# ilovepose/fast-human-pose-estimation.pytorch

Hardware: AMD Instinct MI355X
Metric: images/sec FPD train step (4-stack HG student, 8-stack teacher) 256x256 (higher is better)
Workload: dtype bf16; 1 GPU; configs[1]: hourglass student S=4 F=128 + teacher S=8 F=256, 256x256, batch 32/GPU, fused FPD step incl. Adam, teacher forward one batch ahead on a 2nd stream; global_batch=32, parallelism=dp1, backend=mfma, launch=one native plan call per phase, kernels launched eagerly on 3 streams, ranks=1, finite=True

## Files before the change

### fast-human-pose-estimation.pytorch_amd/csrc/bneck_fused.hip

```cpp
#include <algorithm>
#include <type_traits>

#include "conv_dispatch.h"
#include "fused_lds.h"
#include "fused_tile.h"

namespace {


#ifdef FPD_BNECK_TIMING
#define STAMP(i) do { if (tid == 0 && bid_in == 0) stamps[i] = clock64(); } while (0)
#else
#define STAMP(i) do { } while (0)
#endif

template <int P>
__device__ __forceinline__ void bneck_fold_tables(const fpd_bneck_t& a, float* out, int tid, int nthreads) {
    constexpr int C = 2 * P;
    for (int c = tid; c < C; c += nthreads) {
        float sc, sh;
        bn_coef_eval(a.bn1, c, sc, sh);
        out[c] = sc;
        out[C + c] = sh;
        out[2 * C + 4 * P + c] = a.b3 ? a.b3[c] : 0.f;
    }
    for (int c = tid; c < 2 * P; c += nthreads) {
        const bool second = c >= P;
        const int cc = second ? c - P : c;
        float sc, sh;
        bn_coef_eval(second ? a.bn3 : a.bn2, cc, sc, sh);
        const float* bias = second ? a.b2 : a.b1;
        out[2 * C + (second ? 2 * P : 0) + cc] = sc;
        out[2 * C + (second ? 2 * P : 0) + P + cc] = fmaf(sc, bias ? bias[cc] : 0.f, sh);
    }
}

template <int P>
__global__ void bneck_fold_kernel(const fpd_bneck_t a, float* out) { bneck_fold_tables<P>(a, out, threadIdx.x, blockDim.x); }

template <int P, bool UPADD>
__device__ __forceinline__ void bneck_eval_body(const fpd_bneck_t& a, const int logW, const int bid_in, const int nblk, const int ntiles) {
    using L = BneckLds<P>;
    constexpr int C = L::C, LDX = L::LDX, LD2 = L::LD2, CW = L::CW, ASTG = L::ASTG;
    constexpr int TNH = P / 64;
    constexpr int NSTEP = 9 + 2;
    constexpr int W1V = P * 8 / 512;
    constexpr int NCH = C / 64;
    extern __shared__ __attribute__((aligned(16))) unsigned char smem[];

    const int tid = threadIdx.x, lane = tid & 63, wave = tid >> 6;
#ifdef FPD_BNECK_TIMING
    long long stamps[8];
    long long astamp[10];
    int acnt = 0;
#define ASTAMP() do { if (tid == 0 && bid_in == 0 && acnt < 10) astamp[acnt++] = clock64(); } while (0)
#else
#define ASTAMP() do { } while (0)
#endif
    STAMP(0);
    const int q = wave & 3, hC = wave >> 2;
    const int koff = 8 * (lane >> 5);
    const int H = a.H, W = a.W;
    const int M = a.N * H * W, GR = a.N * H;
    const int nrows = 128 >> logW, hrows = nrows + 2, WP = W + 2;
    const int rrows = 2 * nrows;
    const bool whole = L::whole(H, W);
    const int irows = L::irows(whole, nrows);
    const int zero_px = irows * WP;
    int m0 = 0, g0 = 0;
    int vrow0 = 0;

    float* s_sc1 = reinterpret_cast<float*>(smem);
    float* s_sh1 = s_sc1 + C;
    float* s_sc2 = s_sh1 + C;
    float* s_sh2 = s_sc2 + P;
    float* s_sc3 = s_sh2 + P;
    float* s_sh3 = s_sc3 + P;
    float* s_b3 = s_sh3 + P;
    bf16_t* sA2 = reinterpret_cast<bf16_t*>(s_sc1 + L::TAB);
    bf16_t* sR2 = sA2 + L::image_px(irows, W) * LD2;
    const bf16_t* __restrict__ x = reinterpret_cast<const bf16_t*>(a.x);
    const bf16_t* __restrict__ x2 = reinterpret_cast<const bf16_t*>(UPADD ? a.x2 : nullptr);
    const bf16_t* __restrict__ w1 = reinterpret_cast<const bf16_t*>(a.w1);
    const bf16_t* __restrict__ w2 = reinterpret_cast<const bf16_t*>(a.w2);
    const bf16_t* __restrict__ w3 = reinterpret_cast<const bf16_t*>(a.w3);

    int hp0 = whole ? W : 0;
    int npass = whole ? 1 : ((hrows * W + 127) >> 7);
    const int xpx = tid >> 3, xcv = (tid & 7) * 8;
    int xo[2];
    int xo2[UPADD ? 2 : 1];
    bool xok[2];
    auto pass_addr = [&](int p) __attribute__((always_inline)) {
#pragma unroll
        for (int i = 0; i < 2; ++i) {
            const int hp = hp0 + 128 * p + xpx + 64 * i;
            const int hr = hp >> logW, j = hp & (W - 1);
            const int g = g0 - 1 + hr;
            xok[i] = hr < hrows && (unsigned)g < (unsigned)GR;
            xo[i] = xok[i] ? (g * W + j) * C + xcv : 0;
            if constexpr (UPADD) xo2[i] = xok[i] ? ((((g >> 1) << logW) >> 1) + (j >> 1)) * C + xcv : 0;
        }
    };
    int w1o[W1V], w1l[W1V];
#pragma unroll
    for (int i = 0; i < W1V; ++i) {
        const int v = tid + i * 512;
        w1o[i] = (v >> 3) * C + (v & 7) * 8;
        w1l[i] = 128 * LDX + (v >> 3) * LDX + (v & 7) * 8;
    }
    const int xl = xpx * LDX + xcv;

    u32x4 rx[NCH][2], rw[NCH][W1V];
    u32x4 rx2[UPADD ? NCH : 1][2];
    auto a_load = [&](auto kcc) __attribute__((always_inline)) {
        constexpr int kc = decltype(kcc)::value;
        static_for<2>([&](auto ic) {
            constexpr int i = decltype(ic)::value;
            const u32x4 z = {0u, 0u, 0u, 0u};
            rx[kc][i] = z;
            if (xok[i]) rx[kc][i] = *reinterpret_cast<const u32x4*>(x + (xo[i] + kc * 64));
            if constexpr (UPADD) {
                rx2[kc][i] = z;
                if (xok[i]) rx2[kc][i] = *reinterpret_cast<const u32x4*>(x2 + (xo2[i] + kc * 64));
            }
        });
        static_for<W1V>([&](auto ic) {
            constexpr int i = decltype(ic)::value;
            rw[kc][i] = *reinterpret_cast<const u32x4*>(w1 + (w1o[i] + kc * 64));
        });
    };
    auto a_sum = [&](auto kcc, auto ic) __attribute__((always_inline)) {
        constexpr int kc = decltype(kcc)::value, i = decltype(ic)::value;
        if constexpr (UPADD) rx[kc][i] = bf16x8_sum(rx[kc][i], rx2[kc][i]);
    };
    constexpr int NSL = 2 + W1V;
    auto a_store_slice = [&](auto kcc, auto slc) __attribute__((always_inline)) {
        constexpr int kc = decltype(kcc)::value, sl = decltype(slc)::value;
        bf16_t* dst = sR2 + (kc & 1) * ASTG;
        if constexpr (sl < 2) {
            f32x4 sc[2], sh[2];
            sc[0] = *reinterpret_cast<const f32x4*>(s_sc1 + kc * 64 + xcv);
            sc[1] = *reinterpret_cast<const f32x4*>(s_sc1 + kc * 64 + xcv + 4);
            sh[0] = *reinterpret_cast<const f32x4*>(s_sh1 + kc * 64 + xcv);
            sh[1] = *reinterpret_cast<const f32x4*>(s_sh1 + kc * 64 + xcv + 4);
            float f[8];
            const u32x4 r = rx[kc][sl];
            DT<bf16_t>::unpack(make_uint4(r[0], r[1], r[2], r[3]), f);
#pragma unroll
            for (int e = 0; e < 8; ++e) f[e] = fmaxf(fmaf(f[e], sc[e >> 2][e & 3], sh[e >> 2][e & 3]), 0.f);
            *reinterpret_cast<uint4*>(dst + xl + 64 * sl * LDX) = DT<bf16_t>::pack(f);
        } else if constexpr (sl < NSL) {
            *reinterpret_cast<u32x4*>(dst + w1l[sl - 2]) = rw[kc][sl - 2];
        }
    };
    auto a_store = [&](auto kcc) __attribute__((always_inline)) {
        static_for<NSL>([&](auto slc) { a_store_slice(kcc, slc); });
    };
    constexpr int CPR = P / 8;
    constexpr int RPI = 64 / CPR;
    constexpr int DPW = P / RPI / 8;
    unsigned dma2[DPW], dma3[DPW];
#pragma unroll
    for (int j = 0; j < DPW; ++j) {
        const int row = wave * DPW * RPI + j * RPI + lane / CPR;
        const int sw = (P == 128) ? (row & 15) : ((row >> 1) & 7);
        const int c8 = ((lane % CPR) ^ sw) * 8;
        dma2[j] = (unsigned)(row * 9 * P + c8) * 2u;
        dma3[j] = (unsigned)(row * P + c8) * 2u;
    }
    auto t_dma = [&](auto sc_) __attribute__((always_inline)) {
        constexpr int s = decltype(sc_)::value;
        unsigned char* ring = reinterpret_cast<unsigned char*>(sR2) + (s & 1) * L::RING * 2 + wave * DPW * 1024;
        const char* gbase = s < 9 ? reinterpret_cast<const char*>(w2) + s * P * 2
                                  : reinterpret_cast<const char*>(w3) + (s - 9) * P * P * 2;
        static_for<DPW>([&](auto jc) {
            constexpr int j = decltype(jc)::value;
            unsigned off = s < 9 ? dma2[j] : dma3[j];
            asm volatile("" : "+v"(off));
            __builtin_amdgcn_global_load_lds((const __attribute__((address_space(1))) void*)(gbase + off),
                                             (__attribute__((address_space(3))) void*)(ring + j * 1024), 16, 0, 0);
        });
    };

    if (a.folded != nullptr) {
        for (int v = tid; v < L::TAB / 4; v += 512)
            reinterpret_cast<f32x4*>(s_sc1)[v] = reinterpret_cast<const f32x4*>(a.folded)[v];
    } else {
        bneck_fold_tables<P>(a, s_sc1, tid, 512);
    }

    const int t_beg = fpd_cut(bid_in, ntiles, nblk), t_end = fpd_cut(bid_in + 1, ntiles, nblk);
    for (int tile = t_beg; tile < t_end; ++tile) {
    {
        m0 = tile * 128;
        g0 = m0 >> logW;
        vrow0 = (tile * nrows) % rrows;
        if (!whole) {
            const bool incr = tile > t_beg && (g0 % H) != 0;
            hp0 = incr ? 2 * W : 0;
            npass = incr ? 1 : ((hrows * W + 127) >> 7);
        }
    }
    pass_addr(0);
    static_for<NCH>([&](auto kcc) { a_load(kcc); });
    if (npass > 1) pass_addr(1);
    __syncthreads();
    {
        constexpr int VR = LD2 / 8;
        const uint4 z = make_uint4(0, 0, 0, 0);
        for (int v = tid; v < (2 * irows + 3) * VR; v += 512) {
            const int pz = v / VR, cv = (v - pz * VR) * 8;
            const int px = pz < 2 * irows ? ((pz >> 1) * WP + ((pz & 1) ? WP - 1 : 0)) : zero_px + (pz - 2 * irows);
            *reinterpret_cast<uint4*>(sA2 + px * LD2 + cv) = z;
        }
    }
    a_sum(std::integral_constant<int, 0>{}, std::integral_constant<int, 0>{});
    a_sum(std::integral_constant<int, 0>{}, std::integral_constant<int, 1>{});
    STAMP(1);

    auto refill = [&](auto kcc, int pp) __attribute__((always_inline)) {
        if (pp + 1 < npass) a_load(kcc);
    };
#ifdef FPD_BNECK_TIMING
    acnt = 0;
#endif
    ASTAMP();
    a_store(std::integral_constant<int, 0>{});
    refill(std::integral_constant<int, 0>{}, 0);
    __syncthreads();
    ASTAMP();
    for (int p = 0; p < npass; ++p) {
        f32x16 acc[TNH];
#pragma unroll
        for (int tn = 0; tn < TNH; ++tn)
#pragma unroll
            for (int i = 0; i < 16; ++i) acc[tn][i] = 0.f;
        static_for<NCH>([&](auto kcc) {
            constexpr int kc = decltype(kcc)::value;
            auto stage_slice = [&](auto slc, auto lastc) __attribute__((always_inline)) {
                constexpr bool last = decltype(lastc)::value;
                if constexpr (kc + 1 < NCH) {
                    a_store_slice(std::integral_constant<int, (kc + 1) % NCH>{}, slc);
                    if constexpr (last) refill(std::integral_constant<int, (kc + 1) % NCH>{}, p);
                } else {
                    if (p + 1 < npass) {
                        a_store_slice(std::integral_constant<int, 0>{}, slc);
                        if constexpr (last) {
                            if (p + 2 < npass) pass_addr(p + 2);
                            refill(std::integral_constant<int, 0>{}, p + 1);
                        }
                    }
                }
            };
            const bf16_t* xrow = sR2 + (kc & 1) * ASTG + (q * 32 + (lane & 31)) * LDX + koff;
            const bf16_t* wrow = sR2 + (kc & 1) * ASTG + 128 * LDX + (hC * CW + (lane & 31)) * LDX + koff;
            static_for<4>([&](auto kkc) {
                constexpr int kk = decltype(kkc)::value;
                const bf16x8 px = *reinterpret_cast<const bf16x8*>(xrow + kk * 16);
#pragma unroll
                for (int tn = 0; tn < TNH; ++tn) {
                    const bf16x8 wf = *reinterpret_cast<const bf16x8*>(wrow + tn * 32 * LDX + kk * 16);
                    acc[tn] = __builtin_amdgcn_mfma_f32_32x32x16_bf16(wf, px, acc[tn], 0, 0, 0);
                }
                if constexpr (!UPADD) {
                    stage_slice(kkc, std::integral_constant<bool, kk == NSL - 1>{});
                } else {
                    if constexpr (kk < 2) {
                        if constexpr (kc + 1 < NCH) {
                            if (p == 0) a_sum(std::integral_constant<int, (kc + 1) % NCH>{}, kkc);
                        }
                        stage_slice(std::integral_constant<int, (kk + 2 < NSL ? kk + 2 : NSL)>{}, std::false_type{});
                    } else {
                        stage_slice(std::integral_constant<int, kk - 2>{}, std::integral_constant<bool, kk == 3>{});
                        if (p + 1 < npass) a_sum(kcc, std::integral_constant<int, kk - 2>{});
                    }
                }
            });
            __syncthreads();
            ASTAMP();
        });
        if (p + 1 == npass) {
            t_dma(std::integral_constant<int, 0>{});
            t_dma(std::integral_constant<int, 1>{});
        }
        const int hp = hp0 + 128 * p + q * 32 + (lane & 31);
        const int hr = hp >> logW, j = hp & (W - 1);
        if (hr < hrows) {
            const int rr = whole ? hr : ((vrow0 + hr) & (rrows - 1));
            act_store(acc, s_sc2, s_sh2, hC * CW, lane, sA2 + (rr * WP + j + 1) * LD2);
        }
    }

    const int ml = q * 32 + (lane & 31);
    const int a3px = whole ? 0 : vrow0 * WP;
    int ab[3];
    {
        const int ti = ml >> logW, tj = ml & (W - 1);
        const int g = g0 + ti;
        const int pr = g % H;
        const bool live = g < GR;
        const int r0 = whole ? ti : ((vrow0 + ti) & (rrows - 1)), r1 = whole ? ti + 1 : ((vrow0 + ti + 1) & (rrows - 1)),
                  r2 = whole ? ti + 2 : ((vrow0 + ti + 2) & (rrows - 1));
        ab[0] = (live && pr - 1 >= 0) ? (r0 * WP + tj) * LD2 : zero_px * LD2;
        ab[1] = live ? (r1 * WP + tj) * LD2 : zero_px * LD2;
        ab[2] = (live && pr + 1 < H) ? (r2 * WP + tj) * LD2 : zero_px * LD2;
    }
    STAMP(2);
    __syncthreads();
    STAMP(3);

    f32x16 accB[TNH], accC[2][TNH];
#pragma unroll
    for (int tn = 0; tn < TNH; ++tn)
#pragma unroll
        for (int i = 0; i < 16; ++i) accB[tn][i] = 0.f;

    const int wsw = (P == 128) ? (lane & 15) : ((lane >> 1) & 7);
    auto mma = [&](const bf16_t* arow, int buf, f32x16* acc, auto behind) __attribute__((always_inline)) {
        const bf16_t* wbase = sR2 + buf * L::RING + (hC * CW + (lane & 31)) * P;
        static_for<P / 16>([&](auto kkc) {
            constexpr int kk = decltype(kkc)::value;
            const bf16x8 px = *reinterpret_cast<const bf16x8*>(arow + kk * 16);
            const int wo = ((2 * kk + (lane >> 5)) ^ wsw) * 8;
#pragma unroll
            for (int tn = 0; tn < TNH; ++tn) {
                const bf16x8 wf = *reinterpret_cast<const bf16x8*>(wbase + tn * 32 * P + wo);
                acc[tn] = __builtin_amdgcn_mfma_f32_32x32x16_bf16(wf, px, acc[tn], 0, 0, 0);
            }
            behind(kkc);
        });
    };

    constexpr int VW = CW / 8;
    constexpr int NIT = 32 * VW / 64;
    u32x4 rres[2][NIT];
    u32x4 rres2[UPADD ? NIT : 1];
    auto res_load = [&](auto stc) __attribute__((always_inline)) {
        constexpr int st = decltype(stc)::value;
        static_for<NIT>([&](auto itc) {
            constexpr int it = decltype(itc)::value;
            const int idx = lane + 64 * it;
            const int px = idx / VW, cv = (idx - px * VW) * 8;
            const int m = m0 + q * 32 + px;
            const u32x4 z = {0u, 0u, 0u, 0u};
            rres[st][it] = z;
            if (m < M) rres[st][it] = *reinterpret_cast<const u32x4*>(x + ((size_t)m * C + st * P + hC * CW + cv));
            if constexpr (UPADD) {
                const int g = m >> logW, j = m & (W - 1);
                const int m2 = (((g >> 1) << logW) >> 1) + (j >> 1);
                rres2[it] = z;
                if (m < M) rres2[it] = *reinterpret_cast<const u32x4*>(x2 + ((size_t)m2 * C + st * P + hC * CW + cv));
            }
        });
    };
    auto res_sum = [&](auto stc, auto itc) __attribute__((always_inline)) {
        constexpr int st = decltype(stc)::value, it = decltype(itc)::value;
        if constexpr (UPADD && it < NIT) rres[st][it] = bf16x8_sum(rres[st][it], rres2[it]);
    };

    static_for<NSTEP>([&](auto sc_) {
        constexpr int s = decltype(sc_)::value;
        if constexpr (s >= 1 && s + 1 < NSTEP) t_dma(std::integral_constant<int, (s + 1 < NSTEP ? s + 1 : 0)>{});
        if constexpr (s < 9) {
            mma(sA2 + ab[s / 3] + (s % 3) * LD2 + koff, s & 1, accB, [](auto) {});
        } else {
#pragma unroll
            for (int tn = 0; tn < TNH; ++tn)
#pragma unroll
                for (int i = 0; i < 16; ++i) accC[s - 9][tn][i] = 0.f;
            mma(sA2 + (a3px + ml) * LD2 + koff, s & 1, accC[s - 9],
                [&](auto kkc) { res_sum(std::integral_constant<int, s - 9>{}, kkc); });
        }
        if constexpr (s + 1 < NSTEP) {
            if constexpr (s == 8) res_load(std::integral_constant<int, 0>{});
            if constexpr (s == 9) res_load(std::integral_constant<int, 1>{});
            __syncthreads();
        }
        if constexpr (s == 8) {
            STAMP(4);
            act_store(accB, s_sc3, s_sh3, hC * CW, lane, sA2 + (a3px + ml) * LD2);
            __syncthreads();
        }
    });

    STAMP(5);
    float* stage = reinterpret_cast<float*>(sR2) + wave * 32 * L::LST;
    bf16_t* __restrict__ y = reinterpret_cast<bf16_t*>(a.y);
    static_for<2>([&](auto stc) {
        constexpr int st = decltype(stc)::value;
        __syncthreads();
        epi_stage<TNH>(accC[st], stage, lane);
        __syncthreads();
        static_for<NIT>([&](auto itc) {
            constexpr int it = decltype(itc)::value;
            const int idx = lane + 64 * it;
            const int px = idx / VW, cv = (idx - px * VW) * 8;
            const int m = m0 + q * 32 + px;
            if (m < M) {
                const int c = st * P + hC * CW + cv;
                *reinterpret_cast<uint4*>(y + ((size_t)m * C + c)) = epi_vec(stage + px * L::LST + cv, s_b3 + c, rres[st][it]);
            }
        });
    });
    }
#ifdef FPD_BNECK_TIMING
    STAMP(6);
    if (tid == 0 && bid_in == 0)
        printf("bneck W=%d: setup %lld | phaseA %lld | tile0 %lld | B(9 taps) %lld | a3+C %lld | epilogue %lld | total %lld cycles\n",
               W, stamps[1] - stamps[0], stamps[2] - stamps[1], stamps[3] - stamps[2], stamps[4] - stamps[3],
               stamps[5] - stamps[4], stamps[6] - stamps[5], stamps[6] - stamps[0]);
    if (tid == 0 && bid_in == 0 && acnt == 10)
        printf("  phase A steps: first-stage %lld | pass0 %lld %lld %lld %lld | pass1 %lld %lld %lld %lld | a2 write %lld\n",
               astamp[1] - astamp[0], astamp[2] - astamp[1], astamp[3] - astamp[2], astamp[4] - astamp[3], astamp[5] - astamp[4],
               astamp[6] - astamp[5], astamp[7] - astamp[6], astamp[8] - astamp[7], astamp[9] - astamp[8], stamps[2] - astamp[9]);
#endif
}

template <int P, bool UPADD>
__global__ __launch_bounds__(512, 1) void bneck_eval_kernel(const fpd_bneck_t a, const int logW, const int ntiles) {
    bneck_eval_body<P, UPADD>(a, logW, blockIdx.x, gridDim.x, ntiles);
}

template <int P>
__global__ __launch_bounds__(512, 1) void bneck_eval_pair_kernel(const fpd_bneck_t a, const fpd_bneck_t b, const int logWa,
                                                                 const int logWb, const int nblk_a, const int ntiles_a,
                                                                 const int ntiles_b) {
    if ((int)blockIdx.x < nblk_a) bneck_eval_body<P, false>(a, logWa, blockIdx.x, nblk_a, ntiles_a);
    else bneck_eval_body<P, false>(b, logWb, (int)blockIdx.x - nblk_a, (int)gridDim.x - nblk_a, ntiles_b);
}

static GridCap g_bneck_cap{"FPD_BNECK_BLOCKS", 128};

template <int P>
int launch_bneck_pair(const fpd_bneck_t& a, const fpd_bneck_t& b, hipStream_t st) {
    const size_t lds = std::max(BneckLds<P>::bytes(a.H, a.W), BneckLds<P>::bytes(b.H, b.W));
    static LdsAttr configured;
    if (int rc_ = configured.ensure(reinterpret_cast<const void*>(&bneck_eval_pair_kernel<P>), lds)) return rc_;
    int la = 0, lb = 0;
    while ((1 << la) < a.W) ++la;
    while ((1 << lb) < b.W) ++lb;
    const int ta = cdiv(a.N * a.H * a.W, 128), tb = cdiv(b.N * b.H * b.W, 128);
    int na = ta, nb = tb;
    const int cap = g_bneck_cap.get();
    if (ta + tb > cap) {
        const int capb = std::max(1, (int)((int64_t)cap * tb / (ta + tb)));
        nb = fpd_balanced_blocks(tb, capb);
        na = fpd_balanced_blocks(ta, std::max(1, cap - nb));
    }
    FPD_LAUNCH((bneck_eval_pair_kernel<P>), dim3(na + nb), dim3(512), lds, st, a, b, la, lb, na, ta, tb);
    return 0;
}

template <int P, bool UPADD>
int launch_bneck(const fpd_bneck_t& a, int logW, hipStream_t st) {
    const size_t lds = BneckLds<P>::bytes(a.H, a.W);
    static LdsAttr configured;
    if (int rc_ = configured.ensure(reinterpret_cast<const void*>(&bneck_eval_kernel<P, UPADD>), lds)) return rc_;
    const int ntiles = cdiv(a.N * a.H * a.W, 128);
    FPD_LAUNCH((bneck_eval_kernel<P, UPADD>), dim3(fpd_balanced_blocks(ntiles, g_bneck_cap.get())), dim3(512), lds, st, a, logW, ntiles);
    return 0;
}

}

int fpd_bneck_blocks_option(int value) { return g_bneck_cap.set(value); }

static bool bneck_in_domain(const fpd_bneck_t& a) {
    if (a.dtype != FPD_BF16 || a.C != 2 * a.P || (a.P != 64 && a.P != 128)) return false;
    if (a.W < 4 || a.W > 64 || (a.W & (a.W - 1)) != 0) return false;
    const int hw = a.H * a.W;
    return hw % 128 == 0 || 128 % hw == 0;
}

static EnvOpt g_bneck_upadd{"FPD_BNECK_UPADD", 1};
int fpd_bneck_upadd_option(int value) { return g_bneck_upadd.set(value < 0 ? 0 : value); }

const char* fpd_bneck_upadd_why_not(const fpd_bneck_t& a) {
    if (g_bneck_upadd.get() == 0) return "switched off (FPD_BNECK_UPADD=0 / option bneck_upadd)";
    if (!bneck_in_domain(a)) return "the shape is outside the fused kernel's domain";
    if (a.W < 8) return "W must be one of 8, 16, 32, 64";
    if (a.H & 1) return "H must be even";
    return nullptr;
}

int fpd_bneck_fused_launch(const fpd_bneck_t& a, hipStream_t st) {
    if (!bneck_in_domain(a)) return 1;
    int logW = 0;
    while ((1 << logW) < a.W) ++logW;
    if (a.x2 != nullptr) {
        if (fpd_bneck_upadd_why_not(a) != nullptr) return 1;
        return a.P == 128 ? launch_bneck<128, true>(a, logW, st) : launch_bneck<64, true>(a, logW, st);
    }
    return a.P == 128 ? launch_bneck<128, false>(a, logW, st) : launch_bneck<64, false>(a, logW, st);
}

int fpd_bneck_fused_pair_launch(const fpd_bneck_t& a, const fpd_bneck_t& b, hipStream_t st) {
    if (!bneck_in_domain(a) || !bneck_in_domain(b) || a.P != b.P || a.x2 != nullptr || b.x2 != nullptr) return 1;
    return a.P == 128 ? launch_bneck_pair<128>(a, b, st) : launch_bneck_pair<64>(a, b, st);
}

int fpd_bneck_fold_launch(const fpd_bneck_t& a, float* out, hipStream_t st) {
    if (a.C != 2 * a.P || (a.P != 64 && a.P != 128)) return 1;
    if (a.P == 128) FPD_LAUNCH((bneck_fold_kernel<128>), dim3(1), dim3(256), 0, st, a, out);
    else FPD_LAUNCH((bneck_fold_kernel<64>), dim3(1), dim3(256), 0, st, a, out);
    return 0;
}
```

Measured before the change: 3656 images/s.

## Software-pipeline LDS operand reads ahead of MFMA and use buffer loads for weight DMA

Double-buffers the bf16x8 operand fragments in both the 1x1 conv and the 3x3/1x1 tap loops, so reads for k-step kk+1 (and the next tap's first activation row) are issued before the MFMAs of step kk. sched_group_barrier hints interleave DS reads with MFMAs. The weight DMA switches from global_load_lds to buffer_load_lds with a resource descriptor and constant offsets, which reduces address VALU work. The trade-off is extra VGPR pressure, which is why the UPADD P=128 variant keeps the unpipelined path, and a prefetch across a __syncthreads boundary must read data that is already valid.

Result: no change. 3675 images/s, median of 6 (+0.5%).

```diff
diff --git a/fast-human-pose-estimation.pytorch_amd/csrc/bneck_fused.hip b/fast-human-pose-estimation.pytorch_amd/csrc/bneck_fused.hip
--- a/fast-human-pose-estimation.pytorch_amd/csrc/bneck_fused.hip
+++ b/fast-human-pose-estimation.pytorch_amd/csrc/bneck_fused.hip
@@ -46,6 +46,7 @@
     constexpr int NSTEP = 9 + 2;
     constexpr int W1V = P * 8 / 512;
     constexpr int NCH = C / 64;
+    constexpr bool APIPE = !(UPADD && P == 128);
     extern __shared__ __attribute__((aligned(16))) unsigned char smem[];
 
     const int tid = threadIdx.x, lane = tid & 63, wave = tid >> 6;
@@ -172,14 +173,13 @@
     auto t_dma = [&](auto sc_) __attribute__((always_inline)) {
         constexpr int s = decltype(sc_)::value;
         unsigned char* ring = reinterpret_cast<unsigned char*>(sR2) + (s & 1) * L::RING * 2 + wave * DPW * 1024;
-        const char* gbase = s < 9 ? reinterpret_cast<const char*>(w2) + s * P * 2
-                                  : reinterpret_cast<const char*>(w3) + (s - 9) * P * P * 2;
+        const auto rsrc = __builtin_amdgcn_make_buffer_rsrc(const_cast<bf16_t*>(s < 9 ? w2 : w3), 0, (s < 9 ? 9 * P * P : C * P) * 2, 0x00020000);
         static_for<DPW>([&](auto jc) {
             constexpr int j = decltype(jc)::value;
             unsigned off = s < 9 ? dma2[j] : dma3[j];
             asm volatile("" : "+v"(off));
-            __builtin_amdgcn_global_load_lds((const __attribute__((address_space(1))) void*)(gbase + off),
-                                             (__attribute__((address_space(3))) void*)(ring + j * 1024), 16, 0, 0);
+            __builtin_amdgcn_raw_ptr_buffer_load_lds(rsrc, (__attribute__((address_space(3))) void*)(ring + j * 1024), 16, (int)off,
+                                                     s < 9 ? s * P * 2 : (s - 9) * P * P * 2, 0, 0);
         });
     };
 
@@ -255,14 +255,21 @@
             };
             const bf16_t* xrow = sR2 + (kc & 1) * ASTG + (q * 32 + (lane & 31)) * LDX + koff;
             const bf16_t* wrow = sR2 + (kc & 1) * ASTG + 128 * LDX + (hC * CW + (lane & 31)) * LDX + koff;
+            bf16x8 apx[2], awf[2][TNH];
+            auto a_read = [&](auto kkc) __attribute__((always_inline)) {
+                constexpr int kk = decltype(kkc)::value;
+                apx[kk & 1] = *reinterpret_cast<const bf16x8*>(xrow + kk * 16);
+#pragma unroll
+                for (int tn = 0; tn < TNH; ++tn) awf[kk & 1][tn] = *reinterpret_cast<const bf16x8*>(wrow + tn * 32 * LDX + kk * 16);
+            };
+            if constexpr (APIPE) a_read(std::integral_constant<int, 0>{});
             static_for<4>([&](auto kkc) {
                 constexpr int kk = decltype(kkc)::value;
-                const bf16x8 px = *reinterpret_cast<const bf16x8*>(xrow + kk * 16);
-#pragma unroll
-                for (int tn = 0; tn < TNH; ++tn) {
-                    const bf16x8 wf = *reinterpret_cast<const bf16x8*>(wrow + tn * 32 * LDX + kk * 16);
-                    acc[tn] = __builtin_amdgcn_mfma_f32_32x32x16_bf16(wf, px, acc[tn], 0, 0, 0);
-                }
+                if constexpr (!APIPE) a_read(kkc);
+                else if constexpr (kk + 1 < 4) a_read(std::integral_constant<int, kk + 1>{});
+#pragma unroll
+                for (int tn = 0; tn < TNH; ++tn)
+                    acc[tn] = __builtin_amdgcn_mfma_f32_32x32x16_bf16(awf[kk & 1][tn], apx[kk & 1], acc[tn], 0, 0, 0);
                 if constexpr (!UPADD) {
                     stage_slice(kkc, std::integral_constant<bool, kk == NSL - 1>{});
                 } else {
@@ -317,17 +324,37 @@
         for (int i = 0; i < 16; ++i) accB[tn][i] = 0.f;
 
     const int wsw = (P == 128) ? (lane & 15) : ((lane >> 1) & 7);
-    auto mma = [&](const bf16_t* arow, int buf, f32x16* acc, auto behind) __attribute__((always_inline)) {
+    bf16x8 fpx[2], fwf[2][TNH];
+    auto px_read = [&](const bf16_t* arow, auto kkc) __attribute__((always_inline)) {
+        constexpr int kk = decltype(kkc)::value;
+        fpx[kk & 1] = *reinterpret_cast<const bf16x8*>(arow + kk * 16);
+    };
+    auto w_read = [&](const bf16_t* wbase, auto kkc) __attribute__((always_inline)) {
+        constexpr int kk = decltype(kkc)::value;
+        const int wo = ((2 * kk + (lane >> 5)) ^ wsw) * 8;
+#pragma unroll
+        for (int tn = 0; tn < TNH; ++tn) fwf[kk & 1][tn] = *reinterpret_cast<const bf16x8*>(wbase + tn * 32 * P + wo);
+    };
+    auto mma = [&](const bf16_t* arow, const bf16_t* arow_next, auto own, auto ahead, int buf, f32x16* acc, auto behind) __attribute__((always_inline)) {
         const bf16_t* wbase = sR2 + buf * L::RING + (hC * CW + (lane & 31)) * P;
-        static_for<P / 16>([&](auto kkc) {
+        constexpr int NK = P / 16;
+        if constexpr (decltype(own)::value) px_read(arow, std::integral_constant<int, 0>{});
+        w_read(wbase, std::integral_constant<int, 0>{});
+        __builtin_amdgcn_sched_group_barrier(0x100, TNH + (decltype(own)::value ? 1 : 0), 0);
+        static_for<NK>([&](auto kkc) {
             constexpr int kk = decltype(kkc)::value;
-            const bf16x8 px = *reinterpret_cast<const bf16x8*>(arow + kk * 16);
-            const int wo = ((2 * kk + (lane >> 5)) ^ wsw) * 8;
-#pragma unroll
-            for (int tn = 0; tn < TNH; ++tn) {
-                const bf16x8 wf = *reinterpret_cast<const bf16x8*>(wbase + tn * 32 * P + wo);
-                acc[tn] = __builtin_amdgcn_mfma_f32_32x32x16_bf16(wf, px, acc[tn], 0, 0, 0);
+            if constexpr (kk + 1 < NK) {
+                px_read(arow, std::integral_constant<int, kk + 1>{});
+                w_read(wbase, std::integral_constant<int, kk + 1>{});
+            } else if constexpr (decltype(ahead)::value) {
+                px_read(arow_next, std::integral_constant<int, 0>{});
             }
+#pragma unroll
+            for (int tn = 0; tn < TNH; ++tn)
+                acc[tn] = __builtin_amdgcn_mfma_f32_32x32x16_bf16(fwf[kk & 1][tn], fpx[kk & 1], acc[tn], 0, 0, 0);
+            constexpr int nrd = kk + 1 < NK ? 1 + TNH : (decltype(ahead)::value ? 1 : 0);
+            if constexpr (nrd > 0) __builtin_amdgcn_sched_group_barrier(0x100, nrd, 0);
+            __builtin_amdgcn_sched_group_barrier(0x008, TNH, 0);
             behind(kkc);
         });
     };
@@ -362,14 +389,17 @@
     static_for<NSTEP>([&](auto sc_) {
         constexpr int s = decltype(sc_)::value;
         if constexpr (s >= 1 && s + 1 < NSTEP) t_dma(std::integral_constant<int, (s + 1 < NSTEP ? s + 1 : 0)>{});
+        const bf16_t* a3row = sA2 + (a3px + ml) * LD2 + koff;
         if constexpr (s < 9) {
-            mma(sA2 + ab[s / 3] + (s % 3) * LD2 + koff, s & 1, accB, [](auto) {});
+            constexpr int sn = s + 1 < 9 ? s + 1 : 0;
+            mma(sA2 + ab[s / 3] + (s % 3) * LD2 + koff, sA2 + ab[sn / 3] + (sn % 3) * LD2 + koff, std::integral_constant<bool, s == 0>{},
+                std::integral_constant<bool, (s + 1 < 9)>{}, s & 1, accB, [](auto) {});
         } else {
 #pragma unroll
             for (int tn = 0; tn < TNH; ++tn)
 #pragma unroll
                 for (int i = 0; i < 16; ++i) accC[s - 9][tn][i] = 0.f;
-            mma(sA2 + (a3px + ml) * LD2 + koff, s & 1, accC[s - 9],
+            mma(a3row, a3row, std::integral_constant<bool, s == 9>{}, std::integral_constant<bool, s == 9>{}, s & 1, accC[s - 9],
                 [&](auto kkc) { res_sum(std::integral_constant<int, s - 9>{}, kkc); });
         }
         if constexpr (s + 1 < NSTEP) {
```
